# HKUDS/SSLRec

Hardware: AMD Instinct MI355X
Metric: propagation_edges_per_sec (higher is better)
Workload: dtype f32

## Files before the change

### include/sslrec_hip.h

```cpp
#ifndef SSLREC_HIP_H
#define SSLREC_HIP_H

#include <stddef.h>
#include <stdint.h>

#ifdef __cplusplus
extern "C" {
#endif

#define SSLREC_ABI_VERSION 7
#define SSLREC_E_BADARG 1001

int sslrec_abi_version(void);

int sslrec_row_bits3(const int64_t *idx0, int64_t off0, const int64_t *idx1, int64_t off1, const int64_t *idx2, int64_t off2,
                     int32_t n, int32_t n_rows, uint32_t *bits, void *stream);

typedef struct sslrec_csr {
    int32_t n_rows, n_cols, nnz;
    int32_t d;
    int32_t n_elem;
    const int32_t *col;
    const float   *val;
    int32_t n_waves;
// ... 55 lines not shown
#define SSLREC_SWEPT_LDS_BYTES 163840
typedef struct sslrec_swept {
    int32_t n_rows, n_cols, nnz, d;
    int32_t n_elem, n_blocks, n_slots;
    const int32_t *pack; const float *val;
    const int32_t *w_start, *w_steps;
    const int32_t *wf_ptr;
    const int32_t *cf_ptr;
    const int32_t *f_row, *f_start, *f_n;
} sslrec_swept_t;

int sslrec_swept_deferred_sum_ok(const sslrec_swept_t *A);
int sslrec_spmm_swept_f32(const sslrec_swept_t *A, const int32_t *pack_override, const float *val_override,
                          const int32_t *w_steps_override, const float *X, int32_t d, float *Y,
                          const sslrec_epilogue_t *epi, void *stream);

#define SSLREC_MAX_VIEWS 4
typedef struct sslrec_epilogue_views {
    int32_t n_views; float eps;
    float *Y[SSLREC_MAX_VIEWS];
    const float *noise[SSLREC_MAX_VIEWS];
    const float *acc_in[SSLREC_MAX_VIEWS];
    float *acc_out[SSLREC_MAX_VIEWS];
    const uint64_t *philox;
    uint32_t philox_stream[SSLREC_MAX_VIEWS];
    int32_t philox_noise[SSLREC_MAX_VIEWS];
    const float *row_scale; int32_t scale_flags;
} sslrec_epilogue_views_t;
int sslrec_spmm_swept_views_f32(const sslrec_swept_t *A, const float *X, int32_t d,
                                const sslrec_epilogue_views_t *views, void *stream);
// ... 252 lines not shown
```

### sslrec_amd/_lib.py

```python
import ctypes as C
import os
import subprocess

_HERE = os.path.dirname(os.path.abspath(__file__))
CSRC = os.path.join(_HERE, 'csrc')
SO_PATH = os.environ.get('SSLREC_HIP_LIBRARY') or os.path.join(CSRC, 'libsslrec_hip.so')

E_BADARG = 1001
EXPECTED_ABI = 7


class CsrStruct(C.Structure):
    _fields_ = [
        ('n_rows', C.c_int32), ('n_cols', C.c_int32), ('nnz', C.c_int32), ('d', C.c_int32), ('n_elem', C.c_int32),
        ('col', C.c_void_p), ('val', C.c_void_p),
        ('n_waves', C.c_int32),
        ('w_start', C.c_void_p), ('w_len', C.c_void_p), ('r_ptr', C.c_void_p),
        ('n_rseg', C.c_int32),
        ('r_len', C.c_void_p), ('r_dst', C.c_void_p),
        ('n_long', C.c_int32),
        ('long_row', C.c_void_p), ('long_ptr', C.c_void_p),
        ('n_slots', C.c_int32),
    ]

# ... 31 lines not shown

class EpilogueViewsStruct(C.Structure):
    _fields_ = [('n_views', C.c_int32), ('eps', C.c_float), ('Y', C.c_void_p * 4), ('noise', C.c_void_p * 4),
                ('acc_in', C.c_void_p * 4), ('acc_out', C.c_void_p * 4),
                ('philox', C.c_void_p), ('philox_stream', C.c_uint32 * 4), ('philox_noise', C.c_int32 * 4),
                ('row_scale', C.c_void_p), ('scale_flags', C.c_int32)]


class EpilogueStruct(C.Structure):
    _fields_ = [('noise', C.c_void_p), ('eps', C.c_float), ('acc_in', C.c_void_p), ('acc_out', C.c_void_p),
                ('philox', C.c_void_p), ('philox_stream', C.c_uint32),
                ('noise_sumsq', C.c_void_p), ('noise_row_stride', C.c_int32), ('noise_col_off', C.c_int32),
                ('axpy_x', C.c_void_p), ('axpy_alpha', C.c_float), ('axpy_scale', C.c_void_p), ('x_row_bits', C.c_void_p),
                ('n_sum_in', C.c_int32), ('sum_in', C.c_void_p * 3),
                ('row_scale', C.c_void_p), ('scale_flags', C.c_int32)]


_P = C.c_void_p
_I = C.c_int32
_F = C.c_float

SIGNATURES = {
    'sslrec_abi_version': (C.c_int, []),
    'sslrec_row_bits3': (C.c_int, [_P, C.c_int64, _P, C.c_int64, _P, C.c_int64, _I, _I, _P, _P]),
    'sslrec_debug_stamp_next_launch': (C.c_int, [C.c_void_p]),
    'sslrec_debug_wall_clock_khz': (C.c_int, []),
    'sslrec_philox_row_sumsq': (C.c_int, [_P, C.c_uint32, _I, _I, _P, _P]),
    'sslrec_row_sumsq_f32': (C.c_int, [_P, _I, _I, _P, _P]),
    'sslrec_debug_gather_rows': (C.c_int, [_P, C.c_uint32, _I, _I, _I, _P, _P, _P]),
    'sslrec_debug_swept_trace': (C.c_int, [C.c_int, _P, C.c_int]),
    'sslrec_spmm_csr_f32': (C.c_int, [C.POINTER(CsrStruct), _P, _P, _P, _P, _P, _I, _P, C.POINTER(EpilogueStruct), _P, _P]),
    'sslrec_spmm_bundled_f32': (C.c_int, [C.POINTER(BundledStruct), _P, _P, _I, _P, C.POINTER(EpilogueStruct), _P, _P]),
    'sslrec_spmm_swept_f32': (C.c_int, [C.POINTER(SweptStruct), _P, _P, _P, _P, _I, _P, C.POINTER(EpilogueStruct), _P]),
    'sslrec_swept_deferred_sum_ok': (C.c_int, [C.POINTER(SweptStruct)]),
    'sslrec_spmm_swept_views_f32': (C.c_int, [C.POINTER(SweptStruct), _P, _I, C.POINTER(EpilogueViewsStruct), _P]),
    'sslrec_swept_compact': (C.c_int, [C.POINTER(SweptStruct), _P, _P, _F, _P, _P, _P, _P]),
    'sslrec_edge_drop_compact': (C.c_int, [C.POINTER(CsrStruct), _P, _P, _F, _P, _P, _P, _P, _P]),
    'sslrec_full_predict_f32': (C.c_int, [_P, _P, _I, _P, _I, _I, _P, _I, _P, _P]),
    'sslrec_eval_topk_ws_bytes': (C.c_size_t, [_I, _I, _I]),
    'sslrec_eval_topk_f32': (C.c_int, [_P, _P, _I, _P, _I, _I, _P, _P, _I, _P, _P, _P, _P]),
    'sslrec_sample_negs': (C.c_int, [_P, C.c_int64, _P, _P, _I, _P, C.c_uint32, _P, _P]),
    'sslrec_sample_negs_mt19937': (C.c_int, [_P, _P, _P, C.c_int64, _P, _P, _I, _I, _P, _P]),
    'sslrec_philox_advance': (C.c_int, [_P, _P]),
    'sslrec_philox_fill_f32': (C.c_int, [_P, C.c_uint32, _P, C.c_size_t, _P]),
    'sslrec_mt19937_uniform_f32': (C.c_int, [_P, _P, C.c_int64, _P]),
    'sslrec_mt19937_keep_mask': (C.c_int, [_P, C.c_float, _P, C.c_int64, _P]),
    'sslrec_mt19937_jump_poly': (C.c_int, [_P, _P, _P, _P]),
    'sslrec_mt19937_par_ws_bytes': (C.c_size_t, [C.c_int32, C.c_int32]),
    'sslrec_mt19937_uniform_par_f32': (C.c_int, [_P, _P, C.c_int32, C.c_int32, C.c_int64, _P, _P, C.c_int64, _P]),
# ... 112 lines not shown
```

### sslrec_amd/csrc/losses.hip

```cpp
#include "common.h"
#include "det_scatter.h"
#include <stdlib.h>

typedef float f32x4 __attribute__((ext_vector_type(4)));

#define BPR_BLOCKS 256

__device__ __forceinline__ float bpr_term(float x, int variant) {
    if (variant == 0) {
        return (x > 20.f) ? x : log1pf(expf(x));
    }
    return -logf(1.f / (1.f + expf(x)));
}

__device__ __forceinline__ float bpr_dterm(float x, int variant) {
    if (variant == 0 && x > 20.f) return 1.f;
    return 1.f / (1.f + expf(-x));
}

__device__ __forceinline__ int64_t row_of(const int64_t *idx, int b) { return idx ? idx[b] : (int64_t)b; }

#if defined(__HIP_DEVICE_COMPILE__) && !defined(__gfx950__) && !defined(__gfx942__)
#error "finish_by_last_block relies on gfx942 / gfx950 atomics completing at the coherence point: use release / acquire on this target"
#endif
#define FIN_GROUPS 64
#define FIN_PART0 (32 * (FIN_GROUPS + 1))
static bool one_launch_reduce() {
    static const bool on = [] { const char *e = getenv("SSLREC_ONE_LAUNCH_REDUCE"); return !(e && e[0] == '0'); }();
    return on;
}

__global__ __launch_bounds__(256) void finish_partials_kernel(const float *ws, int n_blocks, float mul, float div, const float *add_in, float *out) {
    __shared__ float s[256];
    const float *part = ws + FIN_PART0;
    float v = 0.f;
    for (int i = threadIdx.x; i < n_blocks; i += 256) v += part[i];
    s[threadIdx.x] = v;
    __syncthreads();
    for (int o = 128; o > 0; o >>= 1) {
        if ((int)threadIdx.x < o) s[threadIdx.x] += s[threadIdx.x + o];
        __syncthreads();
    }
    if (threadIdx.x == 0) {
        const float r = (mul * s[0]) / div;
        out[0] = r;
        if (add_in) out[1] = r + add_in[0];
    }
}

__device__ __forceinline__ void finish_by_last_block(float *ws, float block_partial, int n_blocks, float mul, float div, const float *add_in,
                                                     float *out, int one_launch) {
    __shared__ float s[256];
    __shared__ int is_last;
    float *part = ws + FIN_PART0;
    if (!one_launch) {
        if (threadIdx.x == 0) part[blockIdx.x] = block_partial;
        return;
    }
    if (threadIdx.x == 0) {
        const int gs = (n_blocks + FIN_GROUPS - 1) / FIN_GROUPS, g = blockIdx.x / gs, n_groups = (n_blocks + gs - 1) / gs;
        const int size_g = min(gs, n_blocks - g * gs);
        (void)__hip_atomic_exchange(part + blockIdx.x, block_partial, __ATOMIC_RELAXED, __HIP_MEMORY_SCOPE_AGENT);
        asm volatile("s_waitcnt vmcnt(0)" ::: "memory");
        int last = 0;
        if (atomicInc(reinterpret_cast<unsigned *>(ws + 32 * (g + 1)), (unsigned)size_g - 1u) == (unsigned)size_g - 1u)
            last = atomicInc(reinterpret_cast<unsigned *>(ws), (unsigned)n_groups - 1u) == (unsigned)n_groups - 1u;
        is_last = last;
    }
    __syncthreads();
    if (!is_last) return;
    if (threadIdx.x < 256) {
        float v = 0.f;
        for (int i = threadIdx.x; i < n_blocks; i += 256) v += __hip_atomic_load(part + i, __ATOMIC_RELAXED, __HIP_MEMORY_SCOPE_AGENT);
        s[threadIdx.x] = v;
    }
    __syncthreads();
    for (int o = 128; o > 0; o >>= 1) {
        if ((int)threadIdx.x < o) s[threadIdx.x] += s[threadIdx.x + o];
        __syncthreads();
    }
    if (threadIdx.x == 0) {
        const float r = (mul * s[0]) / div;
        out[0] = r;
        if (add_in) out[1] = r + add_in[0];
    }
}

__global__ __launch_bounds__(256) void bpr_fwd_kernel(const float *Ta, const int64_t *ia, const float *Tp,
                                                      const int64_t *ip, const float *Tn, const int64_t *in,
                                                      int B, int d, int variant, float *ws, float divisor, const float *add_in, float *out,
// ... 708 lines not shown
```

### sslrec_amd/csrc/spmm_swept.hip

```cpp
#include "common.h"
#include "philox.h"
#include "swept_fmt.h"
#include <stdlib.h>
#include <type_traits>

struct SweptArgs {
    const int32_t *pack;
    const float *val;
    const int32_t *w_start, *w_steps;
    const int32_t *wf_ptr, *cf_ptr, *frow, *fstart, *fn;
    int32_t n_slots;
    const float *X;
    int32_t n_views;
    float eps;
    float *Y[SSLREC_MAX_VIEWS];
    const float *noise[SSLREC_MAX_VIEWS];
    const float *acc_in[SSLREC_MAX_VIEWS];
    float *acc_out[SSLREC_MAX_VIEWS];
    const uint64_t *philox;
    uint32_t philox_stream[SSLREC_MAX_VIEWS];
    int32_t philox_noise[SSLREC_MAX_VIEWS];
    int32_t row_stride4, col_off4, n_pass;
    const float *noise_sumsq;
    int32_t noise_rs4, noise_co4;
    const uint32_t *x_bits;
    int32_t n_sum_in;
    const float *sum_in[SSLREC_MAX_SUM_IN];
    const float *axpy_x;
    float axpy_alpha;
    const float *axpy_scale;
    unsigned long long *trace;
    unsigned long long *stamp;
    int32_t nt_stores;
    int32_t prio_mode;
    int32_t late_flush;
    const float *row_scale;
    int32_t scale_flags;
    int32_t acc_init;
};
#define SWEPT_TRACE_MAXB 32

#define SWEPT_WAVES 16

typedef float sw_f32x4 __attribute__((ext_vector_type(4)));

__device__ __forceinline__ void sw_store_sc1(sw_f32x4 *p, sw_f32x4 v) {
    asm volatile("global_store_dwordx4 %0, %1, off sc1" ::"v"(p), "v"(v) : "memory");
}

template <int D, bool PASSES, int WPE, bool PAT>
__global__ __launch_bounds__(1024, WPE) void spmm_swept_kernel(SweptArgs a) {
    extern __shared__ float4 acc[];
    constexpr int G = 256 / D;
    constexpr int LPG = 64 / G;
    constexpr int RV = D / 4;
    constexpr int S = SweptFmt<D>::S;
    const int tid = threadIdx.x;
    const int lane = tid & 63;
    const int sub = lane % LPG;
    const float4 zero4 = make_float4(0.f, 0.f, 0.f, 0.f);
    stamp_begin(a.stamp);

    const int wid = blockIdx.x * SWEPT_WAVES + wave_in_block();
    const int nblk = a.w_steps[wid] / S;
    const int32_t *pl = a.pack + a.w_start[wid] + lane;
// ... 198 lines not shown
        }
    }
    if (a.prio_mode) __builtin_amdgcn_s_setprio(0);
    SW_TRACE_AT(SWEPT_TRACE_MAXB - 3)

    auto sum_in_rows = [&](float4 sa, const size_t at) {
        float4 e[SSLREC_MAX_SUM_IN];
#pragma unroll
        for (int j = 0; j < SSLREC_MAX_SUM_IN; ++j)
            e[j] = j < a.n_sum_in ? reinterpret_cast<const float4 *>(a.sum_in[j])[at] : zero4;
#pragma unroll
        for (int j = 0; j < SSLREC_MAX_SUM_IN; ++j)
            if (j < a.n_sum_in) { sa.x += e[j].x; sa.y += e[j].y; sa.z += e[j].z; sa.w += e[j].w; }
        return sa;
    };
    auto flush_row = [&](const int row, const int s0, const int n, auto have_acc_tag, const float4 acc_row, const float rsc) {
        constexpr bool have_acc = decltype(have_acc_tag)::value;
        const bool live = row >= 0;
        float4 t = zero4;
        size_t at = 0;
        if (live) {
            t = acc[s0 * RV + rs];
            for (int k = 1; k < n; ++k) {
                const float4 w = acc[(s0 + k) * RV + rs];
                t.x += w.x; t.y += w.y; t.z += w.z; t.w += w.w;
            }
            at = (size_t)row * RS + CO + rs;
        }
        if constexpr (PAT) { t.x *= rsc; t.y *= rsc; t.z *= rsc; t.w *= rsc; }
        for (int k = 0; k < a.n_views; ++k) {
            float4 tk = t;
            if (a.noise[k] || a.philox_noise[k]) {
// ... 26 lines not shown
            if (!live) continue;
            if (a.Y[k]) {
                const float ysc = (a.scale_flags & SSLREC_SCALE_Y) ? rsc : 1.f;
                const sw_f32x4 yv = sw_f32x4{tk.x * ysc, tk.y * ysc, tk.z * ysc, tk.w * ysc};
                if (a.nt_stores == 1) __builtin_nontemporal_store(yv, reinterpret_cast<sw_f32x4 *>(a.Y[k]) + at);
                else if (a.nt_stores == 2) sw_store_sc1(reinterpret_cast<sw_f32x4 *>(a.Y[k]) + at, yv);
                else reinterpret_cast<sw_f32x4 *>(a.Y[k])[at] = yv;
            }
            if (a.acc_out[k]) {
                float4 sa = acc_row;
                if constexpr (!have_acc) {
                    sa = reinterpret_cast<const float4 *>(a.acc_in[k])[at];
                    if constexpr (WPE == 4)
                        if (a.n_sum_in) sa = sum_in_rows(sa, at);
                }
                sa.x += tk.x; sa.y += tk.y; sa.z += tk.z; sa.w += tk.w;
                if (a.axpy_x) {
                    const float al = a.axpy_alpha * (a.axpy_scale ? *a.axpy_scale : 1.f);
                    const float4 xr = reinterpret_cast<const float4 *>(a.axpy_x)[at];
                    sa.x = fmaf(al, xr.x, sa.x); sa.y = fmaf(al, xr.y, sa.y); sa.z = fmaf(al, xr.z, sa.z); sa.w = fmaf(al, xr.w, sa.w);
                }
                const float asc = (a.scale_flags & SSLREC_SCALE_ACC) ? rsc : 1.f;
                sa.x *= asc; sa.y *= asc; sa.z *= asc; sa.w *= asc;
                if (a.nt_stores == 1) __builtin_nontemporal_store(sw_f32x4{sa.x, sa.y, sa.z, sa.w}, reinterpret_cast<sw_f32x4 *>(a.acc_out[k]) + at);
                else if (a.nt_stores == 2) sw_store_sc1(reinterpret_cast<sw_f32x4 *>(a.acc_out[k]) + at, sw_f32x4{sa.x, sa.y, sa.z, sa.w});
                else reinterpret_cast<float4 *>(a.acc_out[k])[at] = sa;
            }
        }
    };
#define SW_LDS_BARRIER() asm volatile("s_waitcnt lgkmcnt(0)\n\ts_barrier" ::: "memory")
    if (a.late_flush) SW_LDS_BARRIER();
    typedef std::integral_constant<bool, true> AccGiven;
    typedef std::integral_constant<bool, false> AccRead;
    const float *__restrict__ rsv = a.row_scale;
    float rscp[PFA];
#pragma unroll
    for (int u = 0; u < PFW; ++u) rscp[u] = 1.f;
    if (rsv) {
#pragma unroll
        for (int u = 0; u < PFW; ++u) rscp[u] = rsv[frp[u] == -1 ? 0 : (frp[u] & 0xFFFFF)];
    }
    if (pre_acc && a.n_sum_in == 0) {
        float4 accp[PFA];
#pragma unroll
        for (int u = 0; u < PFW; ++u) {
            accp[u] = zero4;
            if (frp[u] != -1 && !ainit) accp[u] = reinterpret_cast<const float4 *>(a.acc_in[0])[(size_t)SW_FR_ROW(u) * RS + CO + rs];
        }
#pragma unroll
        for (int u = 0; u < PFW; ++u)
            if (u < wpasses) flush_row(SW_FR_ROW(u), SW_FR_S0(u), 1, AccGiven(), accp[u], rscp[u]);
    } else if (pre_acc) {
        constexpr int CH = 3;
#pragma unroll
        for (int u0 = 0; u0 < PFW; u0 += CH) {
            float4 base[CH], e[SSLREC_MAX_SUM_IN][CH];
#pragma unroll
// ... 39 lines not shown
        }
#pragma unroll
        for (int u = 0; u < FU; ++u)
            if (it0 + u < wpasses) flush_row(rowv[u], s0v[u], 1, AccRead(), zero4, rscv[u]);
    }
    if constexpr (WPE != 4)
        if (cf0 + crl < cf1) { crow = a.frow[cf0 + crl]; cs0 = a.fstart[cf0 + crl]; cn = a.fn[cf0 + crl]; }
    float4 cacc = zero4;
    float crsc = 1.f;
    if (rsv) crsc = rsv[crow >= 0 ? crow : 0];
    if constexpr (WPE == 4) {
        if (pre_acc && crow >= 0) {
            const size_t at = (size_t)crow * RS + CO + rs;
            cacc = reinterpret_cast<const float4 *>(a.acc_in[0])[at];
            if (a.n_sum_in) cacc = sum_in_rows(cacc, at);
        }
    }
    if (!a.late_flush) SW_LDS_BARRIER();
    SW_TRACE_AT(SWEPT_TRACE_MAXB - 2)
    if (cpasses > 0) {
        if (WPE == 4 && pre_acc) flush_row(crow, cs0, cn, AccGiven(), cacc, crsc);
        else flush_row(crow, cs0, cn, AccRead(), zero4, crsc);
    }
    for (int it = 1; it < cpasses; ++it) {
        const int i = cf0 + it * RPP + crl;
        const bool live = i < cf1;
        const int row_i = live ? a.frow[i] : -1;
        flush_row(row_i, live ? a.fstart[i] : 0, live ? a.fn[i] : 0, AccRead(), zero4, (rsv && row_i >= 0) ? rsv[row_i] : 1.f);
    }
    SW_TRACE_AT(SWEPT_TRACE_MAXB - 1)
    stamp_end<true>(a.stamp);
}

#define SWEPT_TRACE_RING 4
static unsigned long long *g_swept_trace = nullptr;
static size_t g_swept_trace_stride = 0;
static unsigned g_swept_trace_launch = 0;
extern "C" int sslrec_debug_swept_trace(int enable, unsigned long long *host_out, int n_waves) {
    const size_t stride = (size_t)n_waves * SWEPT_TRACE_MAXB;
    if (enable && !g_swept_trace) {
        if (hipMalloc((void **)&g_swept_trace, SWEPT_TRACE_RING * stride * 8) != hipSuccess) return SSLREC_E_BADARG;
        (void)hipMemset(g_swept_trace, 0, SWEPT_TRACE_RING * stride * 8);
        g_swept_trace_stride = stride;
        g_swept_trace_launch = 0;
    }
// ... 10 lines not shown
    g_next_stamp = record;
    return 0;
}
extern "C" int sslrec_debug_wall_clock_khz(void) {
    int dev = 0, khz = 0;
    if (hipGetDevice(&dev) != hipSuccess) return -1;
    if (hipDeviceGetAttribute(&khz, hipDeviceAttributeWallClockRate, dev) != hipSuccess) return -1;
    return khz;
}
unsigned long long *sslrec_take_stamp() {
    unsigned long long *r = g_next_stamp;
    g_next_stamp = nullptr;
    return r;
}

template <int D, bool PASSES, int WPE, bool PAT>
static int launch_swept_pat(const SweptArgs &a, int n_blocks, hipStream_t st) {
    const size_t lds = (size_t)a.n_slots * D * 4;
    static bool attr_set[64] = {};
    int dev = 0;
    if (hipGetDevice(&dev) != hipSuccess || dev < 0 || dev >= 64) return SSLREC_E_BADARG;
    if (!attr_set[dev]) {
        hipError_t e = hipFuncSetAttribute((const void *)spmm_swept_kernel<D, PASSES, WPE, PAT>, hipFuncAttributeMaxDynamicSharedMemorySize,
                                           SSLREC_SWEPT_LDS_BYTES);
        if (e != hipSuccess) return (int)e;
        attr_set[dev] = true;
    }
    SweptArgs b = a;
    b.trace = nullptr;
    b.stamp = a.stamp;
    static const int late = [] { const char *e = getenv("SSLREC_SWEPT_LATE_FLUSH"); return (e && atoi(e) != 0) ? 1 : 0; }();
    b.late_flush = late;
    static const int prio = [] { const char *e = getenv("SSLREC_SWEPT_PRIO"); return e ? atoi(e) : 2; }();
    b.prio_mode = prio;
    static const int nts = [] { const char *e = getenv("SSLREC_SWEPT_NT_STORES"); return e ? atoi(e) : 2; }();
    b.nt_stores = nts;
    static const int ainit = [] { const char *e = getenv("SSLREC_SWEPT_ACC_INIT"); return (e && atoi(e) != 0) ? 1 : 0; }();
    b.acc_init = ainit;
    if (g_swept_trace && (size_t)n_blocks * SWEPT_WAVES * SWEPT_TRACE_MAXB <= g_swept_trace_stride)
        b.trace = g_swept_trace + (size_t)(g_swept_trace_launch++ % SWEPT_TRACE_RING) * g_swept_trace_stride;
    hipLaunchKernelGGL((spmm_swept_kernel<D, PASSES, WPE, PAT>), dim3(n_blocks), dim3(1024), lds, st, b);
    SSLREC_LAUNCH_CHECK();
    return 0;
}

template <int D, bool PASSES, int WPE>
static int launch_swept_wpe(const SweptArgs &a, int n_blocks, hipStream_t st) {
    if (a.scale_flags & SSLREC_SCALE_PATTERN) return launch_swept_pat<D, PASSES, WPE, true>(a, n_blocks, st);
    return launch_swept_pat<D, PASSES, WPE, false>(a, n_blocks, st);
}

template <int D, bool PASSES>
static int launch_swept_one(const SweptArgs &a, int n_blocks, hipStream_t st) {
    if (n_blocks > 256 || (size_t)a.n_slots * D * 4 <= SSLREC_SWEPT_LDS_BYTES / 2) {
        if (a.n_sum_in) return SSLREC_E_BADARG;
        return launch_swept_wpe<D, PASSES, 8>(a, n_blocks, st);
// ... 189 lines not shown
    }
}

static bool swept_ok(const sslrec_swept_t *A, const float *X, int d) {
    if (!A || !X || A->d <= 0 || d % A->d != 0 || A->n_blocks <= 0 || A->n_slots <= 0) return false;
    const int n_pass = d / A->d;
    if (n_pass != 1 && n_pass != 2 && n_pass != 4 && n_pass != 8) return false;
    return !((size_t)A->n_slots * A->d * 4 > SSLREC_SWEPT_LDS_BYTES || A->n_cols > (1 << 20) || A->n_slots > 4095);
}

extern "C" int sslrec_swept_deferred_sum_ok(const sslrec_swept_t *A) {
    if (!A || A->d <= 0 || A->n_blocks <= 0 || A->n_slots <= 0) return 0;
    return !(A->n_blocks > 256 || (size_t)A->n_slots * A->d * 4 <= SSLREC_SWEPT_LDS_BYTES / 2);
}

extern "C" int sslrec_spmm_swept_f32(const sslrec_swept_t *A, const int32_t *pack_override, const float *val_override,
                                     const int32_t *w_steps_override, const float *X, int32_t d, float *Y,
                                     const sslrec_epilogue_t *epi, void *stream) {
    if (!swept_ok(A, X, d)) return SSLREC_E_BADARG;
    if (!Y && !(epi && epi->acc_out)) return SSLREC_E_BADARG;
    if (epi && epi->acc_out && !epi->acc_in) return SSLREC_E_BADARG;
    SweptArgs a = {};
    a.pack = pack_override ? pack_override : A->pack;
    a.val = val_override ? val_override : A->val;
    a.w_start = A->w_start;
    a.w_steps = w_steps_override ? w_steps_override : A->w_steps;
    a.wf_ptr = A->wf_ptr; a.cf_ptr = A->cf_ptr; a.frow = A->f_row; a.fstart = A->f_start; a.fn = A->f_n;
    a.stamp = sslrec_take_stamp();
    a.n_slots = A->n_slots;
    a.X = X;
    a.n_views = 1;
    a.eps = epi ? epi->eps : 0.f;
    a.Y[0] = Y;
    a.noise[0] = epi ? epi->noise : nullptr;
    a.acc_in[0] = epi ? epi->acc_in : nullptr;
    a.acc_out[0] = epi ? epi->acc_out : nullptr;
    if (epi && !epi->noise && epi->philox) {
// ... 10 lines not shown
        a.noise_co4 = epi->noise_col_off / 4;
        a.axpy_x = epi->axpy_x; a.axpy_alpha = epi->axpy_alpha; a.axpy_scale = epi->axpy_scale;
        a.x_bits = epi->x_row_bits;
        if (epi->scale_flags & ~(SSLREC_SCALE_PATTERN | SSLREC_SCALE_Y | SSLREC_SCALE_ACC)) return SSLREC_E_BADARG;
        if (epi->scale_flags && !epi->row_scale) return SSLREC_E_BADARG;
        if ((epi->scale_flags & SSLREC_SCALE_PATTERN) && epi->x_row_bits) return SSLREC_E_BADARG;
        a.row_scale = epi->scale_flags ? epi->row_scale : nullptr;
        a.scale_flags = epi->scale_flags;
        if (epi->n_sum_in < 0 || epi->n_sum_in > SSLREC_MAX_SUM_IN || (epi->n_sum_in && !epi->acc_out)) return SSLREC_E_BADARG;
        a.n_sum_in = epi->n_sum_in;
        for (int j = 0; j < epi->n_sum_in; ++j) {
            if (!epi->sum_in[j]) return SSLREC_E_BADARG;
            a.sum_in[j] = epi->sum_in[j];
        }
    }
    return swept_dispatch(a, A, d, (hipStream_t)stream);
}

extern "C" int sslrec_spmm_swept_views_f32(const sslrec_swept_t *A, const float *X, int32_t d,
                                           const sslrec_epilogue_views_t *views, void *stream) {
    if (!swept_ok(A, X, d) || !views || views->n_views < 1 || views->n_views > SSLREC_MAX_VIEWS) return SSLREC_E_BADARG;
    SweptArgs a = {};
    a.pack = A->pack; a.val = A->val; a.w_start = A->w_start; a.w_steps = A->w_steps;
    a.wf_ptr = A->wf_ptr; a.cf_ptr = A->cf_ptr; a.frow = A->f_row; a.fstart = A->f_start; a.fn = A->f_n;
    a.stamp = sslrec_take_stamp();
    a.n_slots = A->n_slots;
    a.X = X;
    a.n_views = views->n_views;
    a.eps = views->eps;
    if (views->scale_flags & ~(SSLREC_SCALE_Y | SSLREC_SCALE_ACC)) return SSLREC_E_BADARG;
    if (views->scale_flags && !views->row_scale) return SSLREC_E_BADARG;
// ... 17 lines not shown
```

### sslrec_amd/ops.py

```python
import ctypes as C
import math
import os

import numpy as np
import torch

from . import _lib
from .graph import BundledLayout, DroppedView, EdgePattern, PropGraph, RevaluedView, graph_of, pattern_of

PROFILE = None
PROFILE_EVERY = 1
_profile_tick = 0


def _profile_this_launch():
    global _profile_tick
    if PROFILE is None:
        return False
    _profile_tick += 1
    return PROFILE_EVERY <= 1 or _profile_tick % PROFILE_EVERY == 0


PROFILE_INFONCE = None

# ... 86 lines not shown
    elif ent[1] != cur:
        if not torch.cuda.is_current_stream_capturing():
            cur.wait_stream(ent[1])
        ent[1] = cur
    return ent[0]


import collections
import threading

_KEPT_WS = collections.OrderedDict()
_KEPT_WS_MAX = 8
_KEPT_WS_LOCK = threading.Lock()
SSLREC_KEPT_SCATTER = os.environ.get('SSLREC_KEPT_SCATTER', '1') != '0'
BPR_STAGED = os.environ.get('SSLREC_BPR_STAGED', '1') != '0'


def _bpr_bwd_ws(device, B, d):
    lib = _lib.load()
    n = lib.sslrec_bpr_bwd_ws_bytes(B, d) // 4 + 1
    if not SSLREC_KEPT_SCATTER or 3 * B > 16384 or d > 256 or B <= 0:
        return torch.empty(n, dtype=torch.float32, device=device), False
    ws = _kept_ws(device, B, d)
    st = ws._sslrec_stage
    if st[1]:
        _lib.check(lib.sslrec_bpr_bwd_table_init(ws.data_ptr(), int(B), int(d), _stream()), 'sslrec_bpr_bwd_table_init')
        st[0], st[1] = st[0] + 1, False
    return ws, True


# ... 45 lines not shown


def _idx(t):
    if t is None:
        return None
    if t.dtype != torch.int64:
        t = t.long()
    return t if t.is_contiguous() else t.contiguous()


def _ptr(t):
    return 0 if t is None else t.data_ptr()


def spmm_raw(adj, x, which='fwd', y=None, noise=None, eps=0.0, acc_in=None, acc_out=None, want_y=True, chained=False,
             noise_sumsq=None, noise_geom=None, axpy=None, x_row_bits=None, sum_in=None, row_scale=None, scale_flags=0):
    view = adj if isinstance(adj, (DroppedView, RevaluedView)) else None
    graph = adj.graph if view is not None else adj
    plan = getattr(graph, which)
    _need_gpu(x)
    x = _f32c(x)
    n, d = x.shape
    if n != plan.n_cols:
        raise ValueError('operand has %d rows, matrix has %d columns' % (n, plan.n_cols))
    if d not in SPMM_DIMS and d not in SPMM_NARROW_DIMS:
        raise ValueError('embedding size %d not supported by the raw HIP SpMM launcher (supported: %s and %s); the ops.spmm / '
                         'ops.propagate_sum wrappers zero-pad other sizes' % (d, SPMM_NARROW_DIMS, SPMM_DIMS))
    if want_y and y is None:
        y = torch.empty((plan.n_rows, d), dtype=torch.float32, device=x.device)
    epi = None
    keep_alive = []
# ... 45 lines not shown
    if swept is not None:
        if view is not None:
            col, val, w_len = view.masked(which, d)
    elif scale_flags:
        raise ValueError('the factorized normalization (scale_flags) is the column-swept kernel\'s')
    else:
        lay = plan.packed(d)
        if view is not None:
            col, val, r_len, w_len = view.compact(which, d)
    prof, ev0, ev1 = _profile_this_launch(), None, None
    if prof:
        ev0, ev1 = torch.cuda.Event(enable_timing=True), torch.cuda.Event(enable_timing=True)
        ev0.record()
    if STAMPS is not None:
        STAMPS.attach_next(swept if swept is not None else lay, d, acc_out is not None, want_y, _entry_frac(view), None, len(sum_in or ()))
    if swept is not None:
        rc = lib.sslrec_spmm_swept_f32(C.byref(swept.c_struct()), _ptr(col), _ptr(val), _ptr(w_len), x.data_ptr(), d,
                                       _ptr(y) if want_y else None,
                                       C.byref(epi) if epi is not None else None, _stream())
        _lib.check(rc, 'sslrec_spmm_swept_f32')
        if PROFILE is not None:
            if prof:
                ev1.record()
            PROFILE.append((ev0, ev1, swept, d, acc_out is not None, want_y, _entry_frac(view),
                            x_row_bits.max_rows if (x_row_bits is not None and epi is not None) else None, len(sum_in or ()),
                            bool(scale_flags & SCALE_PATTERN),
                            {'views': 1, 'perturbed': noise is not None, 'philox': noise is not None and not torch.is_tensor(noise), 'which': which}))
        return y if want_y else None
    if isinstance(lay, BundledLayout):
        rc = lib.sslrec_spmm_bundled_view_f32(C.byref(lay.c_struct()), _ptr(col), _ptr(val), _ptr(r_len), _ptr(w_len), x.data_ptr(), d,
                                              _ptr(y) if want_y else None, C.byref(epi) if epi is not None else None,
                                              _ptr(lay.partial_ws()), _stream())
        _lib.check(rc, 'sslrec_spmm_bundled_view_f32')
    else:
        rc = lib.sslrec_spmm_csr_f32(C.byref(lay.c_struct()), _ptr(col), _ptr(val), _ptr(r_len), _ptr(w_len),
# ... 651 lines not shown


def _row_bits_of(t):
    tag = getattr(t, '_sslrec_row_bits', None)
    if tag is None or tag[1] != t._version or tag[0].n_rows != t.shape[0]:
        return None
    return tag[0]


class _PropagateSumFn(torch.autograd.Function):

    @staticmethod
    def forward(ctx, e0, adj, layer_num, noises, eps, keep_layers, noise_sumsq, noise_geom, reg_weight):
        ctx.adj, ctx.layer_num, ctx.reg_weight = adj, layer_num, reg_weight
        e0 = _f32c(e0)
        reg = ()
        if reg_weight is not None:
            lib = _lib.load()
            ws = _ticket_ws(e0.device, lib.sslrec_sumsq_ws_bytes(), 'sumsq')
            out = torch.empty(1, dtype=torch.float32, device=e0.device)
            _lib.check(lib.sslrec_sumsq_fwd_f32(e0.data_ptr(), e0.numel(), float(reg_weight), ws.data_ptr(), out.data_ptr(), _stream()),
                       'sslrec_sumsq_fwd_f32')
            reg = (out.reshape(()),)
            ctx.save_for_backward(e0)
        layers = [e0] if keep_layers else None
        ctx.row_scale = None
        if layer_num == 0:
            return (e0.clone(),) + reg
        total = torch.empty_like(e0)
        x = e0
        plan_f = (adj.graph if isinstance(adj, (DroppedView, RevaluedView)) else adj).fwd
        lay_f = plan_f.swept(e0.shape[1]) if DEFERRED_SUM and 2 <= layer_num <= MAX_SUM_IN + 1 else None
        deferred = lay_f is not None and bool(_lib.load().sslrec_swept_deferred_sum_ok(C.byref(lay_f.c_struct())))
        rsc = None if (deferred or keep_layers or noise_sumsq is not None or noise_geom is not None) else \
            _chain_scale(adj, e0.shape[1], layer_num, perturbed=noises is not None)
        ctx.row_scale = rsc
        mids = []
        for l in range(layer_num):
            last = (l == layer_num - 1)
            want_y = (not last) or keep_layers
            nz = None if noises is None else noises[l]
            nss = None if noise_sumsq is None else noise_sumsq[l]
            if deferred and not last:
                y = spmm_raw(adj, x, 'fwd', noise=nz, eps=eps, noise_sumsq=nss, noise_geom=noise_geom)
                mids.append(y)
            elif deferred:
                y = spmm_raw(adj, x, 'fwd', noise=nz, eps=eps, acc_in=e0, acc_out=total, want_y=want_y, sum_in=mids,
                             noise_sumsq=nss, noise_geom=noise_geom)
            else:
                y = spmm_raw(adj, x, 'fwd', noise=nz, eps=eps, acc_in=e0 if l == 0 else total, acc_out=total, want_y=want_y,
                             chained=l > 0, noise_sumsq=nss, noise_geom=noise_geom, row_scale=rsc,
                             scale_flags=0 if rsc is None else ((SCALE_PATTERN if l > 0 else 0) | (SCALE_Y if want_y else 0)))
            if keep_layers:
                layers.append(y)
            x = y
        ctx.mark_non_differentiable(*(layers[1:] if keep_layers else []))
        return (total,) + reg + (tuple(layers[1:]) if keep_layers else ())

    @staticmethod
    def backward(ctx, g_total, *rest):
        g_reg = rest[0] if ctx.reg_weight is not None else None
        e0 = ctx.saved_tensors[0] if ctx.reg_weight is not None else None
        if g_total is None:
            return (None if g_reg is None else 2.0 * ctx.reg_weight * g_reg * e0,) + (None,) * 8
        sparse = _row_bits_of(g_total) if SPARSE_GRAD else None
        g_total = _f32c(g_total)
        if ctx.layer_num == 0:
# ... 1017 lines not shown
```

Baseline: 57.34 billion.

## Fuse L2 reg sum-of-squares into first swept SpMM flush; add batched axpy path

```diff
diff --git a/include/sslrec_hip.h b/include/sslrec_hip.h
--- a/include/sslrec_hip.h
+++ b/include/sslrec_hip.h
@@ -93,6 +93,19 @@
 int sslrec_spmm_swept_f32(const sslrec_swept_t *A, const int32_t *pack_override, const float *val_override,
                           const int32_t *w_steps_override, const float *X, int32_t d, float *Y,
                           const sslrec_epilogue_t *epi, void *stream);
+
+#define SSLREC_STEP_SUMSQ 1
+#define SSLREC_STEP_AXPY_BATCH 2
+typedef struct {
+    float *sumsq_ws;
+    float *sumsq_out;
+    float sumsq_weight;
+    int32_t flags;
+} sslrec_swept_step_t;
+int sslrec_swept_step_ok(const sslrec_swept_t *A);
+int sslrec_spmm_swept_step_f32(const sslrec_swept_t *A, const int32_t *pack_override, const float *val_override,
+                               const int32_t *w_steps_override, const float *X, int32_t d, float *Y,
+                               const sslrec_epilogue_t *epi, const sslrec_swept_step_t *step, void *stream);
 
 #define SSLREC_MAX_VIEWS 4
 typedef struct sslrec_epilogue_views {
diff --git a/sslrec_amd/_lib.py b/sslrec_amd/_lib.py
--- a/sslrec_amd/_lib.py
+++ b/sslrec_amd/_lib.py
@@ -69,6 +69,13 @@
                 ('axpy_x', C.c_void_p), ('axpy_alpha', C.c_float), ('axpy_scale', C.c_void_p), ('x_row_bits', C.c_void_p),
                 ('n_sum_in', C.c_int32), ('sum_in', C.c_void_p * 3),
                 ('row_scale', C.c_void_p), ('scale_flags', C.c_int32)]
+
+
+STEP_SUMSQ, STEP_AXPY_BATCH = 1, 2
+
+
+class SweptStepStruct(C.Structure):
+    _fields_ = [('sumsq_ws', C.c_void_p), ('sumsq_out', C.c_void_p), ('sumsq_weight', C.c_float), ('flags', C.c_int32)]
 
 
 _P = C.c_void_p
@@ -88,6 +95,9 @@
     'sslrec_spmm_bundled_f32': (C.c_int, [C.POINTER(BundledStruct), _P, _P, _I, _P, C.POINTER(EpilogueStruct), _P, _P]),
     'sslrec_spmm_swept_f32': (C.c_int, [C.POINTER(SweptStruct), _P, _P, _P, _P, _I, _P, C.POINTER(EpilogueStruct), _P]),
     'sslrec_swept_deferred_sum_ok': (C.c_int, [C.POINTER(SweptStruct)]),
+    'sslrec_swept_step_ok': (C.c_int, [C.POINTER(SweptStruct)]),
+    'sslrec_spmm_swept_step_f32': (C.c_int, [C.POINTER(SweptStruct), _P, _P, _P, _P, _I, _P, C.POINTER(EpilogueStruct),
+                                             C.POINTER(SweptStepStruct), _P]),
     'sslrec_spmm_swept_views_f32': (C.c_int, [C.POINTER(SweptStruct), _P, _I, C.POINTER(EpilogueViewsStruct), _P]),
     'sslrec_swept_compact': (C.c_int, [C.POINTER(SweptStruct), _P, _P, _F, _P, _P, _P, _P]),
     'sslrec_edge_drop_compact': (C.c_int, [C.POINTER(CsrStruct), _P, _P, _F, _P, _P, _P, _P, _P]),
diff --git a/sslrec_amd/csrc/fin_reduce.h b/sslrec_amd/csrc/fin_reduce.h
--- /dev/null
+++ b/sslrec_amd/csrc/fin_reduce.h
@@ -0,0 +1,51 @@
+#pragma once
+#include "common.h"
+
+#if defined(__HIP_DEVICE_COMPILE__) && !defined(__gfx950__) && !defined(__gfx942__)
+#error "finish_by_last_block relies on gfx942 / gfx950 atomics completing at the coherence point: use release / acquire on this target"
+#endif
+#define FIN_GROUPS 64
+#define FIN_PART0 (32 * (FIN_GROUPS + 1))
+
+__device__ __forceinline__ void finish_by_last_block_lds(float *ws, float block_partial, int n_blocks, float mul, float div, const float *add_in,
+                                                         float *out, float *s, int *is_last) {
+    float *part = ws + FIN_PART0;
+    if (threadIdx.x == 0) {
+        const int gs = (n_blocks + FIN_GROUPS - 1) / FIN_GROUPS, g = blockIdx.x / gs, n_groups = (n_blocks + gs - 1) / gs;
+        const int size_g = min(gs, n_blocks - g * gs);
+        (void)__hip_atomic_exchange(part + blockIdx.x, block_partial, __ATOMIC_RELAXED, __HIP_MEMORY_SCOPE_AGENT);
+        asm volatile("s_waitcnt vmcnt(0)" ::: "memory");
+        int last = 0;
+        if (atomicInc(reinterpret_cast<unsigned *>(ws + 32 * (g + 1)), (unsigned)size_g - 1u) == (unsigned)size_g - 1u)
+            last = atomicInc(reinterpret_cast<unsigned *>(ws), (unsigned)n_groups - 1u) == (unsigned)n_groups - 1u;
+        *is_last = last;
+    }
+    __syncthreads();
+    if (!*is_last) return;
+    if (threadIdx.x < 256) {
+        float v = 0.f;
+        for (int i = threadIdx.x; i < n_blocks; i += 256) v += __hip_atomic_load(part + i, __ATOMIC_RELAXED, __HIP_MEMORY_SCOPE_AGENT);
+        s[threadIdx.x] = v;
+    }
+    __syncthreads();
+    for (int o = 128; o > 0; o >>= 1) {
+        if ((int)threadIdx.x < o) s[threadIdx.x] += s[threadIdx.x + o];
+        __syncthreads();
+    }
+    if (threadIdx.x == 0) {
+        const float r = (mul * s[0]) / div;
+        out[0] = r;
+        if (add_in) out[1] = r + add_in[0];
+    }
+}
+
+__device__ __forceinline__ void finish_by_last_block(float *ws, float block_partial, int n_blocks, float mul, float div, const float *add_in,
+                                                     float *out, int one_launch) {
+    __shared__ float s[256];
+    __shared__ int is_last;
+    if (!one_launch) {
+        if (threadIdx.x == 0) ws[FIN_PART0 + blockIdx.x] = block_partial;
+        return;
+    }
+    finish_by_last_block_lds(ws, block_partial, n_blocks, mul, div, add_in, out, s, &is_last);
+}
diff --git a/sslrec_amd/csrc/losses.hip b/sslrec_amd/csrc/losses.hip
--- a/sslrec_amd/csrc/losses.hip
+++ b/sslrec_amd/csrc/losses.hip
@@ -1,5 +1,6 @@
 #include "common.h"
 #include "det_scatter.h"
+#include "fin_reduce.h"
 #include <stdlib.h>
 
 typedef float f32x4 __attribute__((ext_vector_type(4)));
@@ -20,11 +21,6 @@
 
 __device__ __forceinline__ int64_t row_of(const int64_t *idx, int b) { return idx ? idx[b] : (int64_t)b; }
 
-#if defined(__HIP_DEVICE_COMPILE__) && !defined(__gfx950__) && !defined(__gfx942__)
-#error "finish_by_last_block relies on gfx942 / gfx950 atomics completing at the coherence point: use release / acquire on this target"
-#endif
-#define FIN_GROUPS 64
-#define FIN_PART0 (32 * (FIN_GROUPS + 1))
 static bool one_launch_reduce() {
     static const bool on = [] { const char *e = getenv("SSLREC_ONE_LAUNCH_REDUCE"); return !(e && e[0] == '0'); }();
     return on;
@@ -36,44 +32,6 @@
     float v = 0.f;
     for (int i = threadIdx.x; i < n_blocks; i += 256) v += part[i];
     s[threadIdx.x] = v;
-    __syncthreads();
-    for (int o = 128; o > 0; o >>= 1) {
-        if ((int)threadIdx.x < o) s[threadIdx.x] += s[threadIdx.x + o];
-        __syncthreads();
-    }
-    if (threadIdx.x == 0) {
-        const float r = (mul * s[0]) / div;
-        out[0] = r;
-        if (add_in) out[1] = r + add_in[0];
-    }
-}
-
-__device__ __forceinline__ void finish_by_last_block(float *ws, float block_partial, int n_blocks, float mul, float div, const float *add_in,
-                                                     float *out, int one_launch) {
-    __shared__ float s[256];
-    __shared__ int is_last;
-    float *part = ws + FIN_PART0;
-    if (!one_launch) {
-        if (threadIdx.x == 0) part[blockIdx.x] = block_partial;
-        return;
-    }
-    if (threadIdx.x == 0) {
-        const int gs = (n_blocks + FIN_GROUPS - 1) / FIN_GROUPS, g = blockIdx.x / gs, n_groups = (n_blocks + gs - 1) / gs;
-        const int size_g = min(gs, n_blocks - g * gs);
-        (void)__hip_atomic_exchange(part + blockIdx.x, block_partial, __ATOMIC_RELAXED, __HIP_MEMORY_SCOPE_AGENT);
-        asm volatile("s_waitcnt vmcnt(0)" ::: "memory");
-        int last = 0;
-        if (atomicInc(reinterpret_cast<unsigned *>(ws + 32 * (g + 1)), (unsigned)size_g - 1u) == (unsigned)size_g - 1u)
-            last = atomicInc(reinterpret_cast<unsigned *>(ws), (unsigned)n_groups - 1u) == (unsigned)n_groups - 1u;
-        is_last = last;
-    }
-    __syncthreads();
-    if (!is_last) return;
-    if (threadIdx.x < 256) {
-        float v = 0.f;
-        for (int i = threadIdx.x; i < n_blocks; i += 256) v += __hip_atomic_load(part + i, __ATOMIC_RELAXED, __HIP_MEMORY_SCOPE_AGENT);
-        s[threadIdx.x] = v;
-    }
     __syncthreads();
     for (int o = 128; o > 0; o >>= 1) {
         if ((int)threadIdx.x < o) s[threadIdx.x] += s[threadIdx.x + o];
diff --git a/sslrec_amd/csrc/spmm_swept.hip b/sslrec_amd/csrc/spmm_swept.hip
--- a/sslrec_amd/csrc/spmm_swept.hip
+++ b/sslrec_amd/csrc/spmm_swept.hip
@@ -1,4 +1,5 @@
 #include "common.h"
+#include "fin_reduce.h"
 #include "philox.h"
 #include "swept_fmt.h"
 #include <stdlib.h>
@@ -37,6 +38,8 @@
     const float *row_scale;
     int32_t scale_flags;
     int32_t acc_init;
+    float *ssq_ws, *ssq_out;
+    float ssq_weight;
 };
 #define SWEPT_TRACE_MAXB 32
 
@@ -48,7 +51,10 @@
     asm volatile("global_store_dwordx4 %0, %1, off sc1" ::"v"(p), "v"(v) : "memory");
 }
 
-template <int D, bool PASSES, int WPE, bool PAT>
+#define SW_TAG_NONE 0
+#define SW_TAG_SSQ 1
+#define SW_TAG_AXB 2
+template <int D, bool PASSES, int WPE, bool PAT, int TAG = SW_TAG_NONE>
 __global__ __launch_bounds__(1024, WPE) void spmm_swept_kernel(SweptArgs a) {
     extern __shared__ float4 acc[];
     constexpr int G = 256 / D;
@@ -277,8 +283,12 @@
             if (j < a.n_sum_in) { sa.x += e[j].x; sa.y += e[j].y; sa.z += e[j].z; sa.w += e[j].w; }
         return sa;
     };
+    float ssq = 0.f;
+    typedef std::integral_constant<int, 1> AccAxGiven;
+    float4 ax_row = zero4;
     auto flush_row = [&](const int row, const int s0, const int n, auto have_acc_tag, const float4 acc_row, const float rsc) {
         constexpr bool have_acc = decltype(have_acc_tag)::value;
+        constexpr bool have_ax = std::is_same<decltype(have_acc_tag), AccAxGiven>::value;
         const bool live = row >= 0;
         float4 t = zero4;
         size_t at = 0;
@@ -335,8 +345,16 @@
                     if constexpr (WPE == 4)
                         if (a.n_sum_in) sa = sum_in_rows(sa, at);
                 }
+                if constexpr (TAG == SW_TAG_SSQ) {
+                    ssq = fmaf(sa.x, sa.x, ssq); ssq = fmaf(sa.y, sa.y, ssq); ssq = fmaf(sa.z, sa.z, ssq); ssq = fmaf(sa.w, sa.w, ssq);
+                }
                 sa.x += tk.x; sa.y += tk.y; sa.z += tk.z; sa.w += tk.w;
-                if (a.axpy_x) {
+                if constexpr (TAG == SW_TAG_AXB) {
+                    const float al = a.axpy_alpha * (a.axpy_scale ? *a.axpy_scale : 1.f);
+                    float4 xr = ax_row;
+                    if constexpr (!have_ax) xr = reinterpret_cast<const float4 *>(a.axpy_x)[at];
+                    sa.x = fmaf(al, xr.x, sa.x); sa.y = fmaf(al, xr.y, sa.y); sa.z = fmaf(al, xr.z, sa.z); sa.w = fmaf(al, xr.w, sa.w);
+                } else if (a.axpy_x) {
                     const float al = a.axpy_alpha * (a.axpy_scale ? *a.axpy_scale : 1.f);
                     const float4 xr = reinterpret_cast<const float4 *>(a.axpy_x)[at];
                     sa.x = fmaf(al, xr.x, sa.x); sa.y = fmaf(al, xr.y, sa.y); sa.z = fmaf(al, xr.z, sa.z); sa.w = fmaf(al, xr.w, sa.w);
@@ -361,7 +379,33 @@
 #pragma unroll
         for (int u = 0; u < PFW; ++u) rscp[u] = rsv[frp[u] == -1 ? 0 : (frp[u] & 0xFFFFF)];
     }
-    if (pre_acc && a.n_sum_in == 0) {
+    if (TAG == SW_TAG_AXB && pre_acc && a.n_sum_in == 0) {
+        constexpr int CH = 4;
+#pragma unroll
+        for (int u0 = 0; u0 < PFW; u0 += CH) {
+            float4 base[CH], xr[CH];
+#pragma unroll
+            for (int c = 0; c < CH; ++c) {
+                const int uc = (u0 + c < PFW) ? u0 + c : 0;
+                const int row = (u0 + c < PFW) ? SW_FR_ROW(uc) : -1;
+                const size_t at = (size_t)(row >= 0 ? row : 0) * RS + CO + rs;
+                base[c] = zero4;
+                xr[c] = zero4;
+                if (row >= 0) {
+                    base[c] = reinterpret_cast<const float4 *>(a.acc_in[0])[at];
+                    xr[c] = reinterpret_cast<const float4 *>(a.axpy_x)[at];
+                }
+            }
+#pragma unroll
+            for (int c = 0; c < CH; ++c) {
+                const int uc = (u0 + c < PFW) ? u0 + c : 0;
+                if (u0 + c < PFW && u0 + c < wpasses) {
+                    ax_row = xr[c];
+                    flush_row(SW_FR_ROW(uc), SW_FR_S0(uc), 1, AccAxGiven(), base[c], rscp[uc]);
+                }
+            }
+        }
+    } else if (pre_acc && a.n_sum_in == 0) {
         float4 accp[PFA];
 #pragma unroll
         for (int u = 0; u < PFW; ++u) {
@@ -431,12 +475,14 @@
             const size_t at = (size_t)crow * RS + CO + rs;
             cacc = reinterpret_cast<const float4 *>(a.acc_in[0])[at];
             if (a.n_sum_in) cacc = sum_in_rows(cacc, at);
+            if constexpr (TAG == SW_TAG_AXB) ax_row = reinterpret_cast<const float4 *>(a.axpy_x)[at];
         }
     }
     if (!a.late_flush) SW_LDS_BARRIER();
     SW_TRACE_AT(SWEPT_TRACE_MAXB - 2)
     if (cpasses > 0) {
-        if (WPE == 4 && pre_acc) flush_row(crow, cs0, cn, AccGiven(), cacc, crsc);
+        if (TAG == SW_TAG_AXB && WPE == 4 && pre_acc) flush_row(crow, cs0, cn, AccAxGiven(), cacc, crsc);
+        else if (WPE == 4 && pre_acc) flush_row(crow, cs0, cn, AccGiven(), cacc, crsc);
         else flush_row(crow, cs0, cn, AccRead(), zero4, crsc);
     }
     for (int it = 1; it < cpasses; ++it) {
@@ -446,6 +492,19 @@
         flush_row(row_i, live ? a.fstart[i] : 0, live ? a.fn[i] : 0, AccRead(), zero4, (rsv && row_i >= 0) ? rsv[row_i] : 1.f);
     }
     SW_TRACE_AT(SWEPT_TRACE_MAXB - 1)
+    if constexpr (TAG == SW_TAG_SSQ) {
+        float *sm = reinterpret_cast<float *>(acc);
+        ssq = wave_sum(ssq);
+        SW_LDS_BARRIER();
+        if (lane == 0) sm[wave_in_block()] = ssq;
+        SW_LDS_BARRIER();
+        float part = 0.f;
+        if (tid == 0) {
+#pragma unroll
+            for (int w = 0; w < SWEPT_WAVES; ++w) part += sm[w];
+        }
+        finish_by_last_block_lds(a.ssq_ws, part, gridDim.x, a.ssq_weight, 1.f, nullptr, a.ssq_out, sm + 64, reinterpret_cast<int *>(sm + 32));
+    }
     stamp_end<true>(a.stamp);
 }
 
@@ -486,14 +545,14 @@
     return r;
 }
 
-template <int D, bool PASSES, int WPE, bool PAT>
+template <int D, bool PASSES, int WPE, bool PAT, int TAG = SW_TAG_NONE>
 static int launch_swept_pat(const SweptArgs &a, int n_blocks, hipStream_t st) {
     const size_t lds = (size_t)a.n_slots * D * 4;
     static bool attr_set[64] = {};
     int dev = 0;
     if (hipGetDevice(&dev) != hipSuccess || dev < 0 || dev >= 64) return SSLREC_E_BADARG;
     if (!attr_set[dev]) {
-        hipError_t e = hipFuncSetAttribute((const void *)spmm_swept_kernel<D, PASSES, WPE, PAT>, hipFuncAttributeMaxDynamicSharedMemorySize,
+        hipError_t e = hipFuncSetAttribute((const void *)spmm_swept_kernel<D, PASSES, WPE, PAT, TAG>, hipFuncAttributeMaxDynamicSharedMemorySize,
                                            SSLREC_SWEPT_LDS_BYTES);
         if (e != hipSuccess) return (int)e;
         attr_set[dev] = true;
@@ -511,7 +570,7 @@
     b.acc_init = ainit;
     if (g_swept_trace && (size_t)n_blocks * SWEPT_WAVES * SWEPT_TRACE_MAXB <= g_swept_trace_stride)
         b.trace = g_swept_trace + (size_t)(g_swept_trace_launch++ % SWEPT_TRACE_RING) * g_swept_trace_stride;
-    hipLaunchKernelGGL((spmm_swept_kernel<D, PASSES, WPE, PAT>), dim3(n_blocks), dim3(1024), lds, st, b);
+    hipLaunchKernelGGL((spmm_swept_kernel<D, PASSES, WPE, PAT, TAG>), dim3(n_blocks), dim3(1024), lds, st, b);
     SSLREC_LAUNCH_CHECK();
     return 0;
 }
@@ -731,13 +790,12 @@
     return !(A->n_blocks > 256 || (size_t)A->n_slots * A->d * 4 <= SSLREC_SWEPT_LDS_BYTES / 2);
 }
 
-extern "C" int sslrec_spmm_swept_f32(const sslrec_swept_t *A, const int32_t *pack_override, const float *val_override,
-                                     const int32_t *w_steps_override, const float *X, int32_t d, float *Y,
-                                     const sslrec_epilogue_t *epi, void *stream) {
+static int swept_one_view_args(SweptArgs &a, const sslrec_swept_t *A, const int32_t *pack_override, const float *val_override,
+                               const int32_t *w_steps_override, const float *X, int32_t d, float *Y, const sslrec_epilogue_t *epi) {
     if (!swept_ok(A, X, d)) return SSLREC_E_BADARG;
     if (!Y && !(epi && epi->acc_out)) return SSLREC_E_BADARG;
     if (epi && epi->acc_out && !epi->acc_in) return SSLREC_E_BADARG;
-    SweptArgs a = {};
+    a = SweptArgs{};
     a.pack = pack_override ? pack_override : A->pack;
     a.val = val_override ? val_override : A->val;
     a.w_start = A->w_start;
@@ -778,7 +836,56 @@
             a.sum_in[j] = epi->sum_in[j];
         }
     }
+    return 0;
+}
+
+extern "C" int sslrec_spmm_swept_f32(const sslrec_swept_t *A, const int32_t *pack_override, const float *val_override,
+                                     const int32_t *w_steps_override, const float *X, int32_t d, float *Y,
+                                     const sslrec_epilogue_t *epi, void *stream) {
+    SweptArgs a;
+    const int rc = swept_one_view_args(a, A, pack_override, val_override, w_steps_override, X, d, Y, epi);
+    if (rc != 0) return rc;
     return swept_dispatch(a, A, d, (hipStream_t)stream);
+}
+
+extern "C" int sslrec_swept_step_ok(const sslrec_swept_t *A) {
+#ifdef SSLREC_SWEPT_ACC_INIT
+    return 0;
+#else
+    if (!sslrec_swept_deferred_sum_ok(A)) return 0;
+    if ((size_t)A->n_slots * A->d * 4 > SSLREC_SWEPT_LDS_BYTES || A->n_cols > (1 << 20) || A->n_slots > 4095) return 0;
+    return A->d == 32 || A->d == 64 || A->d == 128 || A->d == 256;
+#endif
+}
+
+template <int TAG, bool PAT>
+static int launch_swept_tagged(const SweptArgs &a, const sslrec_swept_t *A, hipStream_t st) {
+    switch (A->d) {
+        case 32: return launch_swept_pat<32, false, 4, PAT, TAG>(a, A->n_blocks, st);
+        case 64: return launch_swept_pat<64, false, 4, PAT, TAG>(a, A->n_blocks, st);
+        case 128: return launch_swept_pat<128, false, 4, PAT, TAG>(a, A->n_blocks, st);
+        case 256: return launch_swept_pat<256, false, 4, PAT, TAG>(a, A->n_blocks, st);
+        default: return SSLREC_E_BADARG;
+    }
+}
+
+extern "C" int sslrec_spmm_swept_step_f32(const sslrec_swept_t *A, const int32_t *pack_override, const float *val_override,
+                                          const int32_t *w_steps_override, const float *X, int32_t d, float *Y,
+                                          const sslrec_epilogue_t *epi, const sslrec_swept_step_t *step, void *stream) {
+    if (!step || (step->flags != SSLREC_STEP_SUMSQ && step->flags != SSLREC_STEP_AXPY_BATCH)) return SSLREC_E_BADARG;
+    SweptArgs a;
+    const int rc = swept_one_view_args(a, A, pack_override, val_override, w_steps_override, X, d, Y, epi);
+    if (rc != 0) return rc;
+    if (!sslrec_swept_step_ok(A) || d != A->d || !a.acc_out[0] || a.n_sum_in != 0) return SSLREC_E_BADARG;
+    hipStream_t st = (hipStream_t)stream;
+    if (step->flags == SSLREC_STEP_SUMSQ) {
+        if (!step->sumsq_ws || !step->sumsq_out || a.axpy_x || a.x_bits || (a.scale_flags & SSLREC_SCALE_PATTERN)) return SSLREC_E_BADARG;
+        a.ssq_ws = step->sumsq_ws; a.ssq_out = step->sumsq_out; a.ssq_weight = step->sumsq_weight;
+        return launch_swept_tagged<SW_TAG_SSQ, false>(a, A, st);
+    }
+    if (!a.axpy_x) return SSLREC_E_BADARG;
+    if (a.scale_flags & SSLREC_SCALE_PATTERN) return launch_swept_tagged<SW_TAG_AXB, true>(a, A, st);
+    return launch_swept_tagged<SW_TAG_AXB, false>(a, A, st);
 }
 
 extern "C" int sslrec_spmm_swept_views_f32(const sslrec_swept_t *A, const float *X, int32_t d,
diff --git a/sslrec_amd/ops.py b/sslrec_amd/ops.py
--- a/sslrec_amd/ops.py
+++ b/sslrec_amd/ops.py
@@ -124,6 +124,10 @@
 _KEPT_WS_LOCK = threading.Lock()
 SSLREC_KEPT_SCATTER = os.environ.get('SSLREC_KEPT_SCATTER', '1') != '0'
 BPR_STAGED = os.environ.get('SSLREC_BPR_STAGED', '1') != '0'
+REG_IN_FLUSH = os.environ.get('SSLREC_REG_IN_FLUSH', '1') != '0'
+REG_ROUTES = {'flush': 0, 'kernel': 0}
+AXPY_BATCH = os.environ.get('SSLREC_AXPY_BATCH', '0') == '1'
+AXPY_ROUTES = {'batched': 0, 'plain': 0}
 
 
 def _bpr_bwd_ws(device, B, d):
@@ -199,7 +203,7 @@
 
 
 def spmm_raw(adj, x, which='fwd', y=None, noise=None, eps=0.0, acc_in=None, acc_out=None, want_y=True, chained=False,
-             noise_sumsq=None, noise_geom=None, axpy=None, x_row_bits=None, sum_in=None, row_scale=None, scale_flags=0):
+             noise_sumsq=None, noise_geom=None, axpy=None, x_row_bits=None, sum_in=None, row_scale=None, scale_flags=0, reg_sumsq=None):
     view = adj if isinstance(adj, (DroppedView, RevaluedView)) else None
     graph = adj.graph if view is not None else adj
     plan = getattr(graph, which)
@@ -275,11 +279,27 @@
         ev0.record()
     if STAMPS is not None:
         STAMPS.attach_next(swept if swept is not None else lay, d, acc_out is not None, want_y, _entry_frac(view), None, len(sum_in or ()))
-    if swept is not None:
+    if reg_sumsq is not None and (swept is None or epi is None):
+        raise ValueError('reg_sumsq rides on a column-swept launch with an accumulator')
+    step = None
+    if reg_sumsq is not None:
+        step = _lib.SweptStepStruct(reg_sumsq[0].data_ptr(), reg_sumsq[1].data_ptr(), float(reg_sumsq[2]), _lib.STEP_SUMSQ)
+    elif (AXPY_BATCH and axpy is not None and swept is not None and swept.n_pass == 1 and not sum_in
+          and lib.sslrec_swept_step_ok(C.byref(swept.c_struct()))):
+        step = _lib.SweptStepStruct(None, None, 0.0, _lib.STEP_AXPY_BATCH)
+        AXPY_ROUTES['batched'] += 1
+    if axpy is not None and step is None:
+        AXPY_ROUTES['plain'] += 1
+    if swept is not None and step is not None:
+        rc = lib.sslrec_spmm_swept_step_f32(C.byref(swept.c_struct()), _ptr(col), _ptr(val), _ptr(w_len), x.data_ptr(), d,
+                                            _ptr(y) if want_y else None, C.byref(epi), C.byref(step), _stream())
+        _lib.check(rc, 'sslrec_spmm_swept_step_f32')
+    elif swept is not None:
         rc = lib.sslrec_spmm_swept_f32(C.byref(swept.c_struct()), _ptr(col), _ptr(val), _ptr(w_len), x.data_ptr(), d,
                                        _ptr(y) if want_y else None,
                                        C.byref(epi) if epi is not None else None, _stream())
         _lib.check(rc, 'sslrec_spmm_swept_f32')
+    if swept is not None:
         if PROFILE is not None:
             if prof:
                 ev1.record()
@@ -961,13 +981,25 @@
     def forward(ctx, e0, adj, layer_num, noises, eps, keep_layers, noise_sumsq, noise_geom, reg_weight):
         ctx.adj, ctx.layer_num, ctx.reg_weight = adj, layer_num, reg_weight
         e0 = _f32c(e0)
-        reg = ()
+        plan_f = (adj.graph if isinstance(adj, (DroppedView, RevaluedView)) else adj).fwd
+        lay_f = plan_f.swept(e0.shape[1]) if DEFERRED_SUM and 2 <= layer_num <= MAX_SUM_IN + 1 else None
+        deferred = lay_f is not None and bool(_lib.load().sslrec_swept_deferred_sum_ok(C.byref(lay_f.c_struct())))
+        reg, reg_ride = (), None
         if reg_weight is not None:
             lib = _lib.load()
             ws = _ticket_ws(e0.device, lib.sslrec_sumsq_ws_bytes(), 'sumsq')
             out = torch.empty(1, dtype=torch.float32, device=e0.device)
-            _lib.check(lib.sslrec_sumsq_fwd_f32(e0.data_ptr(), e0.numel(), float(reg_weight), ws.data_ptr(), out.data_ptr(), _stream()),
-                       'sslrec_sumsq_fwd_f32')
+            lay_r = None
+            if (REG_IN_FLUSH and layer_num >= 1 and noises is None and not keep_layers and noise_sumsq is None and noise_geom is None
+                    and not deferred):
+                lay_r = plan_f.swept(e0.shape[1])
+            if lay_r is not None and lay_r.n_pass == 1 and lib.sslrec_swept_step_ok(C.byref(lay_r.c_struct())):
+                reg_ride = (ws, out, float(reg_weight))
+                REG_ROUTES['flush'] += 1
+            else:
+                _lib.check(lib.sslrec_sumsq_fwd_f32(e0.data_ptr(), e0.numel(), float(reg_weight), ws.data_ptr(), out.data_ptr(), _stream()),
+                           'sslrec_sumsq_fwd_f32')
+                REG_ROUTES['kernel'] += 1
             reg = (out.reshape(()),)
             ctx.save_for_backward(e0)
         layers = [e0] if keep_layers else None
@@ -976,9 +1008,6 @@
             return (e0.clone(),) + reg
         total = torch.empty_like(e0)
         x = e0
-        plan_f = (adj.graph if isinstance(adj, (DroppedView, RevaluedView)) else adj).fwd
-        lay_f = plan_f.swept(e0.shape[1]) if DEFERRED_SUM and 2 <= layer_num <= MAX_SUM_IN + 1 else None
-        deferred = lay_f is not None and bool(_lib.load().sslrec_swept_deferred_sum_ok(C.byref(lay_f.c_struct())))
         rsc = None if (deferred or keep_layers or noise_sumsq is not None or noise_geom is not None) else \
             _chain_scale(adj, e0.shape[1], layer_num, perturbed=noises is not None)
         ctx.row_scale = rsc
@@ -997,7 +1026,8 @@
             else:
                 y = spmm_raw(adj, x, 'fwd', noise=nz, eps=eps, acc_in=e0 if l == 0 else total, acc_out=total, want_y=want_y,
                              chained=l > 0, noise_sumsq=nss, noise_geom=noise_geom, row_scale=rsc,
-                             scale_flags=0 if rsc is None else ((SCALE_PATTERN if l > 0 else 0) | (SCALE_Y if want_y else 0)))
+                             scale_flags=0 if rsc is None else ((SCALE_PATTERN if l > 0 else 0) | (SCALE_Y if want_y else 0)),
+                             reg_sumsq=reg_ride if l == 0 else None)
             if keep_layers:
                 layers.append(y)
             x = y
```

Measured after the change: 58.18 billion, median of 6. 1.5% higher.
